# ritikasaboo13/Quantized-GEMM-for-Transformer-Inference

Measured on AMD Instinct MI355X. Metric: int8 GEMMs/sec + achieved int8-MFMA TOPS%, M=N=K=4096, 1/2/4/8 MI355X, higher is better.
Workload: dtype int8

## Files before the change

### include/qgemm.h

```cpp
#ifndef QGEMM_H_
#define QGEMM_H_

#include <stddef.h>
#include <stdint.h>

#if defined(__GNUC__)
#define QGEMM_API __attribute__((visibility("default")))
#else
#define QGEMM_API
#endif

#ifdef __cplusplus
extern "C" {
#endif

QGEMM_API int op_mm_quantize(const float *A, const float *B, float *C, int m, int n, int k);

QGEMM_API int op_mm_quantize_ex(const float *A, int64_t a_stride_h, int64_t a_stride_w,
                      const float *B, int64_t b_stride_h, int64_t b_stride_w,
                      float *C, int64_t c_stride_h, int64_t c_stride_w,
                      int m, int n, int k, float range, void *stream);

QGEMM_API size_t op_mm_quantize_workspace_size(int m, int n, int k);
QGEMM_API int op_mm_quantize_ws(const float *A, int64_t a_stride_h, int64_t a_stride_w,
// ... 33 lines not shown
QGEMM_API int qgemm_linear_dt(const void *X, int x_dtype, int64_t x_stride_h, int m, int k, const void *packed_w, int n,
                    const float *bias, int relu, void *Y, int y_dtype, int64_t y_stride_h,
                    void *workspace, size_t ws_bytes, void *stream);
QGEMM_API int qgemm_softmax_rows(const float *S, float *P, int64_t rows, int w, float scale, void *stream);
QGEMM_API int qgemm_softmax_rows_causal(const float *S, float *P, int64_t rows, int w, float scale, int seq_q,
                              int q_pos0, void *stream);
QGEMM_API int qgemm_add_layernorm_rows(const float *A, const float *B, float *Y, int64_t rows, int w, void *stream);
QGEMM_API int qgemm_encoder_create(int d_model, int n_heads, int d_ff, int n_blocks, int max_seq, uint64_t seed,
                         void **encoder);
QGEMM_API int qgemm_encoder_forward(void *encoder, const float *X, float *Y, int seq, void *stream);
QGEMM_API int qgemm_encoder_destroy(void *encoder);

QGEMM_API size_t qgemm_attention_workspace_size(int seq_q, int seq_kv, int n_heads, int d_k);
QGEMM_API int qgemm_attention(const float *Q, int64_t q_stride_h, const float *K, int64_t k_stride_h,
                    const float *V, int64_t v_stride_h, float *O, int64_t o_stride_h,
                    int seq_q, int seq_kv, int n_heads, int d_k, float scale,
                    void *workspace, size_t ws_bytes, void *stream);
QGEMM_API int qgemm_attention_causal(const float *Q, int64_t q_stride_h, const float *K, int64_t k_stride_h,
                           const float *V, int64_t v_stride_h, float *O, int64_t o_stride_h,
                           int seq_q, int seq_kv, int n_heads, int d_k, float scale, int q_pos0,
                           void *workspace, size_t ws_bytes, void *stream);
QGEMM_API int qgemm_attention_plan(int seq_q, int seq_kv, int n_heads, int d_k, const char **kernel);

QGEMM_API int qgemm_decoder_create(int d_model, int n_heads, int d_ff, int n_blocks, int max_seq, int max_enc_seq,
                         uint64_t seed, void **decoder);
enum { QGEMM_DECODER_CAUSAL = 1, QGEMM_DECODER_KV_CACHE = 8 };
QGEMM_API int qgemm_decoder_create_ex(int d_model, int n_heads, int d_ff, int n_blocks, int max_seq, int max_enc_seq,
                            uint64_t seed, int flags, void **decoder);
QGEMM_API int qgemm_decoder_forward(void *decoder, const float *X, const float *enc_out, float *Y, int seq, int enc_seq,
                          void *stream);
QGEMM_API int qgemm_decoder_begin(void *decoder, const float *enc_out, int enc_seq, void *stream);
QGEMM_API int qgemm_decoder_step(void *decoder, const float *X, float *Y, int pos, int n, void *stream);
QGEMM_API int qgemm_decoder_destroy(void *decoder);

QGEMM_API size_t qgemm_mm_outlier_workspace_size(int m, int n, int k);
QGEMM_API int qgemm_mm_outlier(const float *A, const float *B, float *C, int m, int n, int k, float threshold,
                     void *workspace, size_t ws_bytes, void *stream);
QGEMM_API int qgemm_outlier_count(int k, const void *workspace, int *count);

QGEMM_API size_t qgemm_linear_outlier_workspace_size(int m, int n, int k);
QGEMM_API int qgemm_linear_outlier(const float *X, int64_t x_stride_h, int m, int k, const void *packed_w, int n,
                         const float *bias, int relu, float threshold, float *Y, int64_t y_stride_h,
                         void *workspace, size_t ws_bytes, void *stream);

QGEMM_API int qgemm_error_stats(const float *C, const float *O, int64_t count, int reference_order, double *stats,
                      void *stream);

QGEMM_API int qgemm_fill_uniform(float *dst, int64_t count, uint64_t seed, float lo, float hi, void *stream);

QGEMM_API int qgemm_set_gemm_events(void *start_event, void *stop_event);
QGEMM_API int qgemm_set_event_mode(int mode);

QGEMM_API int qgemm_gemm_plan(int m, int n, int k, int *tile, const char **kernel);

QGEMM_API const char *qgemm_version(void);

#ifdef __cplusplus
}
#endif

#endif
```

### include/qgemm_dist.h

```cpp
#ifndef QGEMM_DIST_H_
#define QGEMM_DIST_H_

#include <stddef.h>
#include <stdint.h>

#include "qgemm.h"

#ifdef __cplusplus
extern "C" {
#endif

#define QGEMM_COMM_ID_BYTES 128

QGEMM_API int qgemm_shard_rows(int m, int world, int rank, int *m0, int *rows);

QGEMM_API int op_mm_quantize_shard(const float *A, const float *B, float *C, int m, int n, int k, int world,
                                   int rank, void *stream);

QGEMM_API int qgemm_comm_unique_id(void *id_out );
QGEMM_API int qgemm_comm_init_rank(void **comm, int world, const void *id, int rank);
QGEMM_API int qgemm_comm_init_all(void **comms, int ndev, const int *devices);
QGEMM_API int qgemm_comm_destroy(void *comm);
QGEMM_API int qgemm_comm_count(void *comm, int *count);
QGEMM_API int qgemm_comm_user_rank(void *comm, int *rank);

QGEMM_API int qgemm_allgather_rows(float *C, int m, int n, int world, int rank, void *comm, void *stream);
QGEMM_API int qgemm_allgather_plan(int m, int n, int world, int64_t *first, int64_t *count, int *root, int max_ops);

QGEMM_API int qgemm_allgather_chunk_plan(int m, int n, int world, int chunks, int64_t *first, int64_t *count,
                                         int *root, int max_ops);
QGEMM_API size_t op_mm_quantize_shard_pipelined_workspace_size(int m, int n, int k, int world, int chunks);
QGEMM_API int op_mm_quantize_shard_pipelined(const float *A, const float *B, float *C, int m, int n, int k, int world,
                                             int rank, int chunks, void *comm, void *workspace, size_t ws_bytes,
                                             void *stream, void *gather_stream);

typedef struct qgemm_coll_op {
    int rank;
    int root;
    int64_t send_off;
    int64_t recv_off;
    int64_t count;
} qgemm_coll_op;

QGEMM_API int qgemm_node_allgather_plan(int m, int n, int ndev, qgemm_coll_op *ops, int max_ops);

QGEMM_API int qgemm_node_mm_quantize(const float *const *A, const float *const *B, float *const *C, int m, int n,
                                     int k, int ndev, const int *devices, void *const *comms,
                                     void *const *streams, int mode);

#ifdef __cplusplus
}
#endif

#endif
```

### quantized-gemm-for-transformer-inference_amd/__init__.py

```python
from __future__ import annotations

import ctypes
import os
import subprocess
import threading

PKG_DIR = os.path.dirname(os.path.abspath(__file__))
REPO_DIR = os.path.dirname(PKG_DIR)
LIB_PATH = os.path.join(PKG_DIR, "build", "libqgemm.so")
HEADER_PATH = os.path.join(REPO_DIR, "include", "qgemm.h")
DIST_LIB_PATH = os.path.join(PKG_DIR, "build", "libqgemm_dist.so")
DIST_HEADER_PATH = os.path.join(REPO_DIR, "include", "qgemm_dist.h")

DEFAULT_RANGE = 127.0
ROW_PAD = 256
K_PAD = 128

EXPORTED_SYMBOLS = (
    "op_mm_quantize",
    "op_mm_quantize_ex",
    "op_mm_quantize_workspace_size",
    "op_mm_quantize_ws",
    "qgemm_packed_size",
    "qgemm_pack_a",
    "qgemm_pack_b",
    "qgemm_mm_packed",
    "qgemm_mm_packed_i32",
    "qgemm_mm_fp32",
    "qgemm_error_stats",
    "qgemm_linear_workspace_size",
    "qgemm_linear",
    "qgemm_pack_a_dt",
    "qgemm_mm_packed_dt",
    "qgemm_linear_dt",
    "op_mm_quantize_prepacked",
    "op_mm_quantize_prepacked_workspace_size",
    "op_mm_quantize_prepacked_ws",
    "qgemm_softmax_rows",
    "qgemm_softmax_rows_causal",
    "qgemm_add_layernorm_rows",
    "qgemm_encoder_create",
    "qgemm_encoder_forward",
    "qgemm_encoder_destroy",
    "qgemm_attention_workspace_size",
    "qgemm_attention",
    "qgemm_attention_causal",
    "qgemm_attention_plan",
    "qgemm_decoder_create",
    "qgemm_decoder_create_ex",
    "qgemm_decoder_forward",
    "qgemm_decoder_begin",
    "qgemm_decoder_step",
    "qgemm_decoder_destroy",
    "qgemm_mm_outlier_workspace_size",
    "qgemm_mm_outlier",
    "qgemm_outlier_count",
    "qgemm_linear_outlier_workspace_size",
    "qgemm_linear_outlier",
    "qgemm_set_gemm_events",
    "qgemm_set_event_mode",
    "qgemm_fill_uniform",
    "qgemm_gemm_plan",
    "qgemm_version",
)

DIST_EXPORTED_SYMBOLS = (
    "qgemm_shard_rows",
    "op_mm_quantize_shard",
    "qgemm_comm_unique_id",
    "qgemm_comm_init_rank",
    "qgemm_comm_init_all",
    "qgemm_comm_destroy",
    "qgemm_comm_count",
    "qgemm_comm_user_rank",
    "qgemm_allgather_rows",
    "qgemm_allgather_plan",
    "qgemm_allgather_chunk_plan",
    "op_mm_quantize_shard_pipelined_workspace_size",
    "op_mm_quantize_shard_pipelined",
    "qgemm_node_allgather_plan",
    "qgemm_node_mm_quantize",
)
COMM_ID_BYTES = 128

HIP_ERROR_INVALID_VALUE = 1
QGEMM_F32, QGEMM_BF16 = 0, 1
QGEMM_DECODER_CAUSAL = 1
QGEMM_DECODER_KV_CACHE = 8

_lock = threading.Lock()
_lib = None
_dist = None


class QGemmError(RuntimeError):

    def __init__(self, fn: str, code: int):
        super().__init__(f"{fn} failed with hipError_t {code}")
        self.code = code


def build(verbose: bool = False) -> str:
    out = None if verbose else subprocess.DEVNULL
    jobs = str(min(8, os.cpu_count() or 1))
    subprocess.run(["make", "-C", PKG_DIR, "-j", jobs, "all"], check=True, stdout=out)
    return LIB_PATH


def load() -> ctypes.CDLL:
    global _lib
    with _lock:
        if _lib is not None:
            return _lib
        if not os.path.exists(LIB_PATH):
            raise RuntimeError(f"qgemm HIP library not built: {LIB_PATH} missing (run build())")
        L = ctypes.CDLL(LIB_PATH)
        i64, i32, f32, vp, sz = ctypes.c_int64, ctypes.c_int, ctypes.c_float, ctypes.c_void_p, ctypes.c_size_t
        L.op_mm_quantize.argtypes = [vp, vp, vp, i32, i32, i32]
        L.op_mm_quantize.restype = i32
        L.op_mm_quantize_ex.argtypes = [vp, i64, i64, vp, i64, i64, vp, i64, i64, i32, i32, i32, f32, vp]
        L.op_mm_quantize_ex.restype = i32
        L.op_mm_quantize_workspace_size.argtypes = [i32, i32, i32]
        L.op_mm_quantize_workspace_size.restype = sz
        L.op_mm_quantize_ws.argtypes = [vp, i64, i64, vp, i64, i64, vp, i64, i64, i32, i32, i32, f32, vp, sz, vp]
        L.op_mm_quantize_ws.restype = i32
        L.qgemm_packed_size.argtypes = [i32, i32]
        L.qgemm_packed_size.restype = sz
        L.qgemm_pack_a.argtypes = [vp, i64, i64, i32, i32, f32, vp, vp]
        L.qgemm_pack_a.restype = i32
        L.qgemm_pack_b.argtypes = [vp, i64, i64, i32, i32, f32, vp, vp]
        L.qgemm_pack_b.restype = i32
        L.qgemm_mm_packed.argtypes = [vp, vp, vp, i64, i64, i32, i32, i32, f32, vp]
# ... 21 lines not shown
        L.op_mm_quantize_prepacked_ws.argtypes = [vp, i64, vp, vp, i64, i32, i32, i32, vp, sz, vp]
        L.op_mm_quantize_prepacked_ws.restype = i32
        L.qgemm_softmax_rows.argtypes = [vp, vp, i64, i32, f32, vp]
        L.qgemm_softmax_rows.restype = i32
        L.qgemm_softmax_rows_causal.argtypes = [vp, vp, i64, i32, f32, i32, i32, vp]
        L.qgemm_softmax_rows_causal.restype = i32
        L.qgemm_add_layernorm_rows.argtypes = [vp, vp, vp, i64, i32, vp]
        L.qgemm_add_layernorm_rows.restype = i32
        L.qgemm_encoder_create.argtypes = [i32, i32, i32, i32, i32, ctypes.c_uint64, ctypes.POINTER(vp)]
        L.qgemm_encoder_create.restype = i32
        L.qgemm_encoder_forward.argtypes = [vp, vp, vp, i32, vp]
        L.qgemm_encoder_forward.restype = i32
        L.qgemm_encoder_destroy.argtypes = [vp]
        L.qgemm_encoder_destroy.restype = i32
        L.qgemm_attention_workspace_size.argtypes = [i32, i32, i32, i32]
        L.qgemm_attention_workspace_size.restype = sz
        L.qgemm_attention.argtypes = [vp, i64, vp, i64, vp, i64, vp, i64, i32, i32, i32, i32, f32, vp, sz, vp]
        L.qgemm_attention.restype = i32
        L.qgemm_attention_causal.argtypes = [vp, i64, vp, i64, vp, i64, vp, i64, i32, i32, i32, i32, f32, i32, vp, sz,
                                             vp]
        L.qgemm_attention_causal.restype = i32
        L.qgemm_decoder_create_ex.argtypes = [i32, i32, i32, i32, i32, i32, ctypes.c_uint64, i32, ctypes.POINTER(vp)]
        L.qgemm_decoder_create_ex.restype = i32
        L.qgemm_decoder_create.argtypes = [i32, i32, i32, i32, i32, i32, ctypes.c_uint64, ctypes.POINTER(vp)]
        L.qgemm_decoder_create.restype = i32
        L.qgemm_decoder_forward.argtypes = [vp, vp, vp, vp, i32, i32, vp]
        L.qgemm_decoder_forward.restype = i32
        L.qgemm_decoder_begin.argtypes = [vp, vp, i32, vp]
        L.qgemm_decoder_begin.restype = i32
        L.qgemm_decoder_step.argtypes = [vp, vp, vp, i32, i32, vp]
        L.qgemm_decoder_step.restype = i32
        L.qgemm_attention_plan.argtypes = [i32, i32, i32, i32, ctypes.POINTER(ctypes.c_char_p)]
        L.qgemm_attention_plan.restype = i32
        L.qgemm_decoder_destroy.argtypes = [vp]
        L.qgemm_decoder_destroy.restype = i32
        L.qgemm_mm_outlier_workspace_size.argtypes = [i32, i32, i32]
        L.qgemm_mm_outlier_workspace_size.restype = sz
        L.qgemm_mm_outlier.argtypes = [vp, vp, vp, i32, i32, i32, f32, vp, sz, vp]
        L.qgemm_mm_outlier.restype = i32
        L.qgemm_outlier_count.argtypes = [i32, vp, ctypes.POINTER(i32)]
        L.qgemm_outlier_count.restype = i32
        L.qgemm_linear_outlier_workspace_size.argtypes = [i32, i32, i32]
        L.qgemm_linear_outlier_workspace_size.restype = sz
        L.qgemm_linear_outlier.argtypes = [vp, i64, i32, i32, vp, i32, vp, i32, f32, vp, i64, vp, sz, vp]
        L.qgemm_linear_outlier.restype = i32
        L.qgemm_fill_uniform.argtypes = [vp, i64, ctypes.c_uint64, f32, f32, vp]
        L.qgemm_fill_uniform.restype = i32
        L.qgemm_set_gemm_events.argtypes = [vp, vp]
        L.qgemm_set_gemm_events.restype = i32
        L.qgemm_set_event_mode.argtypes = [i32]
        L.qgemm_set_event_mode.restype = i32
        L.qgemm_gemm_plan.argtypes = [i32, i32, i32, ctypes.POINTER(ctypes.c_int), ctypes.POINTER(ctypes.c_char_p)]
        L.qgemm_gemm_plan.restype = i32
        L.qgemm_version.argtypes = []
        L.qgemm_version.restype = ctypes.c_char_p
        _lib = L
        return L


def load_dist() -> ctypes.CDLL:
    global _dist
    load()
    with _lock:
        if _dist is not None:
            return _dist
        if not os.path.exists(DIST_LIB_PATH):
            raise RuntimeError(f"qgemm multi-GPU library not built: {DIST_LIB_PATH} missing (run build())")
        D = ctypes.CDLL(DIST_LIB_PATH)
        i32, vp = ctypes.c_int, ctypes.c_void_p
        D.qgemm_shard_rows.argtypes = [i32, i32, i32, ctypes.POINTER(i32), ctypes.POINTER(i32)]
        D.qgemm_shard_rows.restype = i32
        D.op_mm_quantize_shard.argtypes = [vp, vp, vp, i32, i32, i32, i32, i32, vp]
        D.op_mm_quantize_shard.restype = i32
        D.qgemm_comm_unique_id.argtypes = [vp]
        D.qgemm_comm_unique_id.restype = i32
        D.qgemm_comm_init_rank.argtypes = [ctypes.POINTER(vp), i32, vp, i32]
        D.qgemm_comm_init_rank.restype = i32
        D.qgemm_comm_init_all.argtypes = [ctypes.POINTER(vp), i32, ctypes.POINTER(i32)]
        D.qgemm_comm_init_all.restype = i32
        D.qgemm_comm_destroy.argtypes = [vp]
        D.qgemm_comm_destroy.restype = i32
        D.qgemm_comm_count.argtypes = [vp, ctypes.POINTER(i32)]
        D.qgemm_comm_count.restype = i32
        D.qgemm_comm_user_rank.argtypes = [vp, ctypes.POINTER(i32)]
        D.qgemm_comm_user_rank.restype = i32
        D.qgemm_allgather_rows.argtypes = [vp, i32, i32, i32, i32, vp, vp]
        D.qgemm_allgather_rows.restype = i32
        i64p = ctypes.POINTER(ctypes.c_int64)
        D.qgemm_allgather_plan.argtypes = [i32, i32, i32, i64p, i64p, ctypes.POINTER(i32), i32]
        D.qgemm_allgather_plan.restype = i32
        D.qgemm_allgather_chunk_plan.argtypes = [i32, i32, i32, i32, i64p, i64p, ctypes.POINTER(i32), i32]
        D.qgemm_allgather_chunk_plan.restype = i32
        D.op_mm_quantize_shard_pipelined_workspace_size.argtypes = [i32, i32, i32, i32, i32]
        D.op_mm_quantize_shard_pipelined_workspace_size.restype = ctypes.c_size_t
        D.op_mm_quantize_shard_pipelined.argtypes = [vp, vp, vp, i32, i32, i32, i32, i32, i32, vp, vp, ctypes.c_size_t,
                                                     vp, vp]
        D.op_mm_quantize_shard_pipelined.restype = i32
        D.qgemm_node_allgather_plan.argtypes = [i32, i32, i32, ctypes.POINTER(CollOp), i32]
        D.qgemm_node_allgather_plan.restype = i32
        D.qgemm_node_mm_quantize.argtypes = [vp, vp, vp, i32, i32, i32, i32, ctypes.POINTER(i32), vp, vp, i32]
        D.qgemm_node_mm_quantize.restype = i32
        _dist = D
        return D


def shard_rows(m: int, world: int, rank: int) -> tuple:
    m0, rows = ctypes.c_int(), ctypes.c_int()
    _check("qgemm_shard_rows", load_dist().qgemm_shard_rows(m, world, rank, ctypes.byref(m0), ctypes.byref(rows)))
    return m0.value, rows.value


class CollOp(ctypes.Structure):
    _fields_ = [("rank", ctypes.c_int), ("root", ctypes.c_int), ("send_off", ctypes.c_int64),
                ("recv_off", ctypes.c_int64), ("count", ctypes.c_int64)]


def node_allgather_plan(m: int, n: int, ndev: int) -> list:
    D = load_dist()
    cnt = D.qgemm_node_allgather_plan(m, n, ndev, None, 0)
    if cnt < 0:
        raise QGemmError("qgemm_node_allgather_plan", -cnt)
    ops = (CollOp * max(1, cnt))()
    got = D.qgemm_node_allgather_plan(m, n, ndev, ops, cnt)
    if got != cnt:
        raise QGemmError("qgemm_node_allgather_plan", -got if got < 0 else 1)
    return [(o.rank, o.root, o.send_off, o.recv_off, o.count) for o in ops[:cnt]]


def allgather_plan(m: int, n: int, world: int) -> list:
    cap = max(1, world)
    first, count, root = (ctypes.c_int64 * cap)(), (ctypes.c_int64 * cap)(), (ctypes.c_int * cap)()
    ops = load_dist().qgemm_allgather_plan(m, n, world, first, count, root, cap)
    if ops < 0:
        raise QGemmError("qgemm_allgather_plan", -ops)
    return [(first[i], count[i], root[i]) for i in range(ops)]


def allgather_chunk_plan(m: int, n: int, world: int, chunks: int) -> list:
    D = load_dist()
    cnt = D.qgemm_allgather_chunk_plan(m, n, world, chunks, None, None, None, 0)
    if cnt < 0:
        raise QGemmError("qgemm_allgather_chunk_plan", -cnt)
    cap = max(1, cnt)
    first, count, root = (ctypes.c_int64 * cap)(), (ctypes.c_int64 * cap)(), (ctypes.c_int * cap)()
    got = D.qgemm_allgather_chunk_plan(m, n, world, chunks, first, count, root, cap)
    if got != cnt:
        raise QGemmError("qgemm_allgather_chunk_plan", -got if got < 0 else 1)
    return [(first[i], count[i], root[i]) for i in range(cnt)]


# ... 578 lines not shown
```

### quantized-gemm-for-transformer-inference_amd/csrc/api.hip

```cpp
#include <map>
#include <mutex>
#include <thread>
#include <stdio.h>

#include "../../include/qgemm.h"
#include "qgemm_internal.h"

using namespace qgemm;

namespace {

constexpr float kDefaultRange = 127.0f;

int err(hipError_t e) { return (int)e; }

bool dims_ok(int m, int n, int k) { return m >= 0 && n >= 0 && k >= 1; }

hipError_t pack_vectors(const float *src, int64_t row_stride, int64_t elem_stride, int rows, int len, float range,
                        PackedView out, hipStream_t stream) {
    if (elem_stride == 1) return launch_pack_rows(src, row_stride, 1, rows, len, range, out, stream);
    if (row_stride == 1 && len > 1) return launch_pack_cols(src, elem_stride, len, rows, range, out, stream);
    return launch_pack_rows(src, row_stride, elem_stride, rows, len, range, out, stream);
}

hipError_t pack_vectors(const bf16_t *src, int64_t row_stride, int64_t elem_stride, int rows, int len, float range,
                        PackedView out, hipStream_t stream) {
    return launch_pack_rows(src, row_stride, elem_stride, rows, len, range, out, stream);
}

bool dtype_ok(int t) { return t == QGEMM_F32 || t == QGEMM_BF16; }

hipError_t pack_vectors(const void *src, int dtype, int64_t row_stride, int64_t elem_stride, int rows, int len,
                        float range, PackedView out, hipStream_t stream) {
    return dtype == QGEMM_BF16
               ? pack_vectors(static_cast<const bf16_t *>(src), row_stride, elem_stride, rows, len, range, out, stream)
               : pack_vectors(static_cast<const float *>(src), row_stride, elem_stride, rows, len, range, out, stream);
}

enum CacheUse { kUseWorkspace = 0, kUseSplitK = 1, kUseErrorStats = 2 };
constexpr int kMaxCachedStreams = 8;
struct CacheKey {
    int dev;
    hipStream_t stream;
    std::thread::id thread;
    int use;
    bool operator<(const CacheKey &o) const {
        if (dev != o.dev) return dev < o.dev;
        if (stream != o.stream) return stream < o.stream;
        if (thread != o.thread) return thread < o.thread;
        return use < o.use;
    }
};
// ... 31 lines not shown
    if (e != hipSuccess) return e;
    const std::thread::id th = stream == hipStreamPerThread ? std::this_thread::get_id() : std::thread::id();
    std::lock_guard<std::mutex> lk(g_cache_mu);
    const CacheKey key{dev, stream, th, use};
    const bool fresh = g_cache.find(key) == g_cache.end();
    CachedBuf &w = g_cache[key];
    w.last_use = ++g_cache_clock;
    if (fresh && (e = evict_cached(dev, use, key)) != hipSuccess) return e;
    if (w.bytes < need) {
        if (w.ptr) {
            if ((e = hipStreamSynchronize(stream)) != hipSuccess) return e;
            if ((e = hipFree(w.ptr)) != hipSuccess) return e;
            w.ptr = nullptr;
            w.bytes = 0;
        }
        const size_t grow = need + headroom;
        if ((e = hipMalloc(&w.ptr, grow)) != hipSuccess) return e;
        if (zero_new && (e = hipMemset(w.ptr, 0, grow)) != hipSuccess) return e;
        w.bytes = grow;
    }
    *out = w.ptr;
    return hipSuccess;
}

hipError_t cached_workspace(size_t need, hipStream_t stream, void **out) {
    return cached_buffer(need, stream, kUseWorkspace, false, need / 8 , out);
}

size_t align256(size_t x) { return (x + 255) & ~(size_t)255; }

struct ChainWorkspace {
    size_t scratch_bytes;
    size_t a, b;
    size_t end;
    ChainWorkspace(int m, int n, int k)
        : scratch_bytes(gemm_scratch_bytes(m, n, k)),
          a(align256(scratch_bytes)),
          b(a + align256(packed_bytes(m, k))),
          end(b + align256(packed_bytes(n, k))) {}
};

hipError_t cached_scratch(size_t need, hipStream_t stream, int use, void **out) {
    return cached_buffer(need, stream, use, true, 0, out);
}

hipError_t mm_packed_impl(const void *packed_a, const void *packed_b, void *C, int64_t c_stride_h,
                          int64_t c_stride_w, int m, int n, int k, float range, void *scratch, size_t scratch_bytes,
                          hipStream_t stream, bool tickets_zeroed = false, bool c_bf16 = false) {
    const float inv_r2 = 1.0f / (range * range);
    return launch_gemm_dequant(packed_view(packed_a, m, k), packed_view(packed_b, n, k), C, c_stride_h, c_stride_w, m,
                               n, inv_r2, scratch, scratch_bytes, stream, nullptr, false, tickets_zeroed, c_bf16);
}

}

extern "C" {

size_t qgemm_packed_size(int rows, int k) {
    if (rows < 0 || k < 1) return 0;
    return packed_bytes(rows, k);
}

size_t op_mm_quantize_workspace_size(int m, int n, int k) {
    if (!dims_ok(m, n, k)) return 0;
    return ChainWorkspace(m, n, k).end;
}

int qgemm_pack_a(const float *A, int64_t a_stride_h, int64_t a_stride_w, int m, int k, float range, void *packed_a,
                 void *stream) {
    return qgemm_pack_a_dt(A, QGEMM_F32, a_stride_h, a_stride_w, m, k, range, packed_a, stream);
}

int qgemm_pack_b(const float *B, int64_t b_stride_h, int64_t b_stride_w, int k, int n, float range, void *packed_b,
                 void *stream) {
    if (!B || !packed_b || n < 0 || k < 1) return err(hipErrorInvalidValue);
    if (n == 0) return 0;
    return err(pack_vectors(B, b_stride_w, b_stride_h, n, k, range, packed_view(packed_b, n, k),
                            static_cast<hipStream_t>(stream)));
}

int qgemm_mm_packed(const void *packed_a, const void *packed_b, float *C, int64_t c_stride_h, int64_t c_stride_w,
                    int m, int n, int k, float range, void *stream) {
    return qgemm_mm_packed_dt(packed_a, packed_b, C, QGEMM_F32, c_stride_h, c_stride_w, m, n, k, range, stream);
}

int qgemm_mm_packed_i32(const void *packed_a, const void *packed_b, int32_t *Acc, int m, int n, int k, void *stream) {
    if (!packed_a || !packed_b || !Acc || !dims_ok(m, n, k)) return err(hipErrorInvalidValue);
    if (m == 0 || n == 0) return 0;
    return err(launch_gemm_i32(packed_view(packed_a, m, k), packed_view(packed_b, n, k), Acc, m, n,
                               static_cast<hipStream_t>(stream)));
}

int op_mm_quantize_ws(const float *A, int64_t a_stride_h, int64_t a_stride_w, const float *B, int64_t b_stride_h,
                      int64_t b_stride_w, float *C, int64_t c_stride_h, int64_t c_stride_w, int m, int n, int k,
                      float range, void *workspace, size_t ws_bytes, void *stream) {
    if (!A || !B || !C || !dims_ok(m, n, k)) return err(hipErrorInvalidValue);
    if (m == 0 || n == 0) return 0;
    const ChainWorkspace ws(m, n, k);
    if (!workspace || ws_bytes < ws.end) return err(hipErrorInvalidValue);
    char *scratch = static_cast<char *>(workspace);
    char *pa = scratch + ws.a, *pb = scratch + ws.b;
    hipStream_t s = static_cast<hipStream_t>(stream);
    auto gemm = [&](bool tickets_zeroed) {
        return err(mm_packed_impl(pa, pb, C, c_stride_h, c_stride_w, m, n, k, range, scratch, ws.scratch_bytes, s,
                                  tickets_zeroed));
    };
    uint32_t *tickets = reinterpret_cast<uint32_t *>(scratch);
    const int ntickets = (int)(gemm_ticket_bytes(m, n, k) / 4);
    if (a_stride_w == 1 && b_stride_w == 1 && k > 1) {
        const PackedView va = packed_view(pa, m, k), vb = packed_view(pb, n, k);
        hipError_t e = launch_pack_single_pass(A, a_stride_h, m, k, va, B, b_stride_h, n, vb, range, s, tickets, ntickets);
        if (e == hipSuccess) return gemm(true);
        if (e != hipErrorNotSupported) return err(e);
        e = launch_pack_two_pass(A, a_stride_h, m, k, va, B, b_stride_h, n, vb, range, s, tickets, ntickets);
        if (e == hipSuccess) return gemm(true);
        if (e != hipErrorNotSupported) return err(e);
    }
    int rc = qgemm_pack_a(A, a_stride_h, a_stride_w, m, k, range, pa, stream);
    if (rc) return rc;
    rc = qgemm_pack_b(B, b_stride_h, b_stride_w, k, n, range, pb, stream);
    if (rc) return rc;
    return gemm(false);
}

int op_mm_quantize_ex(const float *A, int64_t a_stride_h, int64_t a_stride_w, const float *B, int64_t b_stride_h,
                      int64_t b_stride_w, float *C, int64_t c_stride_h, int64_t c_stride_w, int m, int n, int k,
                      float range, void *stream) {
    if (!A || !B || !C || !dims_ok(m, n, k)) return err(hipErrorInvalidValue);
    if (m == 0 || n == 0) return 0;
    const size_t need = op_mm_quantize_workspace_size(m, n, k);
    void *ws = nullptr;
    hipError_t e = cached_workspace(need, static_cast<hipStream_t>(stream), &ws);
    if (e != hipSuccess) return err(e);
    return op_mm_quantize_ws(A, a_stride_h, a_stride_w, B, b_stride_h, b_stride_w, C, c_stride_h, c_stride_w, m, n, k,
                             range, ws, need, stream);
}

int op_mm_quantize(const float *A, const float *B, float *C, int m, int n, int k) {
    return op_mm_quantize_ex(A, k, 1, B, n, 1, C, n, 1, m, n, k, kDefaultRange, nullptr);
}

int qgemm_mm_fp32(const float *A, int64_t a_stride_h, int64_t a_stride_w, const float *B, int64_t b_stride_h,
                  int64_t b_stride_w, float *C, int64_t c_stride_h, int64_t c_stride_w, int m, int n, int k,
                  void *stream) {
    if (!A || !B || !C || !dims_ok(m, n, k)) return err(hipErrorInvalidValue);
    if (m == 0 || n == 0) return 0;
    return err(launch_mm_f32(A, a_stride_h, a_stride_w, B, b_stride_h, b_stride_w, C, c_stride_h, c_stride_w, m, n, k,
                             static_cast<hipStream_t>(stream)));
}

int qgemm_error_stats(const float *C, const float *O, int64_t count, int reference_order, double *stats,
                      void *stream) {
    if (!C || !O || !stats || count < 1) return err(hipErrorInvalidValue);
    hipStream_t s = static_cast<hipStream_t>(stream);
    void *scratch = nullptr;
    hipError_t e = cached_scratch(error_stats_scratch_bytes(), s, kUseErrorStats, &scratch);
    if (e != hipSuccess) return err(e);
    return err(launch_error_stats(C, O, count, reference_order != 0, stats, scratch, s));
}

int qgemm_linear(const float *X, int64_t x_stride_h, int m, int k, const void *packed_w, int n, const float *bias,
                 int relu, float *Y, int64_t y_stride_h, void *workspace, size_t ws_bytes, void *stream) {
// ... 282 lines not shown
```

### quantized-gemm-for-transformer-inference_amd/csrc/dist.cpp

```cpp
#include <hip/hip_runtime.h>
#include <rccl/rccl.h>

#include <vector>

#include "../../include/qgemm_dist.h"

namespace {

int nccl_rc(ncclResult_t r) { return r == ncclSuccess ? 0 : 1000 + (int)r; }

}

extern "C" {

int qgemm_shard_rows(int m, int world, int rank, int *m0, int *rows) {
    if (m < 0 || world < 1 || rank < 0 || rank >= world || !m0 || !rows) return (int)hipErrorInvalidValue;
    const int q = m / world, r = m % world;
    *m0 = rank * q + (rank < r ? rank : r);
    *rows = q + (rank < r ? 1 : 0);
    return 0;
}

int op_mm_quantize_shard(const float *A, const float *B, float *C, int m, int n, int k, int world, int rank,
                         void *stream) {
    int m0 = 0, rows = 0;
    const int e = qgemm_shard_rows(m, world, rank, &m0, &rows);
    if (e) return e;
    if (!A || !B || !C || n < 0 || k < 1) return (int)hipErrorInvalidValue;
    if (rows == 0) return 0;
    return op_mm_quantize_ex(A + (int64_t)m0 * k, k, 1, B, n, 1, C + (int64_t)m0 * n, n, 1, rows, n, k, 127.0f,
                             stream);
}

int qgemm_comm_unique_id(void *id_out) {
    if (!id_out) return (int)hipErrorInvalidValue;
    return nccl_rc(ncclGetUniqueId(static_cast<ncclUniqueId *>(id_out)));
}

int qgemm_comm_init_rank(void **comm, int world, const void *id, int rank) {
    if (!comm || !id || world < 1 || rank < 0 || rank >= world) return (int)hipErrorInvalidValue;
    ncclUniqueId uid;
    __builtin_memcpy(&uid, id, sizeof(uid));
    ncclComm_t c = nullptr;
    const int rc = nccl_rc(ncclCommInitRank(&c, world, uid, rank));
    *comm = c;
    return rc;
}

int qgemm_comm_init_all(void **comms, int ndev, const int *devices) {
    if (!comms || ndev < 1) return (int)hipErrorInvalidValue;
    return nccl_rc(ncclCommInitAll(reinterpret_cast<ncclComm_t *>(comms), ndev, devices));
}

int qgemm_comm_destroy(void *comm) {
    if (!comm) return 0;
    return nccl_rc(ncclCommDestroy(static_cast<ncclComm_t>(comm)));
}

int qgemm_comm_count(void *comm, int *count) {
    if (!comm || !count) return (int)hipErrorInvalidValue;
    return nccl_rc(ncclCommCount(static_cast<ncclComm_t>(comm), count));
}

int qgemm_comm_user_rank(void *comm, int *rank) {
    if (!comm || !rank) return (int)hipErrorInvalidValue;
    return nccl_rc(ncclCommUserRank(static_cast<ncclComm_t>(comm), rank));
}

int qgemm_allgather_plan(int m, int n, int world, int64_t *first, int64_t *count, int *root, int max_ops) {
    if (m < 0 || n < 0 || world < 1 || max_ops < 0 || (max_ops > 0 && (!first || !count || !root)))
        return -(int)hipErrorInvalidValue;
    if (world == 1 || m == 0 || n == 0) return 0;
    if (m % world == 0) {
        if (max_ops < 1) return -(int)hipErrorInvalidValue;
        first[0] = 0;
        count[0] = (int64_t)(m / world) * n;
        root[0] = -1;
        return 1;
    }
    int ops = 0;
    for (int r = 0; r < world; ++r) {
        int m0 = 0, rows = 0;
        qgemm_shard_rows(m, world, r, &m0, &rows);
        if (rows == 0) continue;
        if (ops >= max_ops) return -(int)hipErrorInvalidValue;
        first[ops] = (int64_t)m0 * n;
        count[ops] = (int64_t)rows * n;
        root[ops] = r;
        ++ops;
    }
    return ops;
}

namespace {

int chunk_plan(int m, int n, int world, int chunks, int64_t *first, int64_t *count, int *root, int *chunk_of,
               int max_ops) {
    const bool query = first == nullptr;
    int ops = 0;
    for (int c = 0; c < chunks; ++c)
        for (int r = 0; r < world; ++r) {
            int m0 = 0, rows = 0, c0 = 0, crows = 0;
            qgemm_shard_rows(m, world, r, &m0, &rows);
            qgemm_shard_rows(rows, chunks, c, &c0, &crows);
            if (crows == 0 || n == 0) continue;
            if (!query) {
                if (ops >= max_ops) return -(int)hipErrorInvalidValue;
                first[ops] = (int64_t)(m0 + c0) * n;
                count[ops] = (int64_t)crows * n;
                root[ops] = r;
                if (chunk_of) chunk_of[ops] = c;
            }
            ++ops;
        }
    return ops;
}

}

int qgemm_allgather_chunk_plan(int m, int n, int world, int chunks, int64_t *first, int64_t *count, int *root,
                               int max_ops) {
    if (m < 0 || n < 0 || world < 1 || chunks < 1 || max_ops < 0) return -(int)hipErrorInvalidValue;
    if (max_ops == 0 || !first || !count || !root) return chunk_plan(m, n, world, chunks, nullptr, nullptr, nullptr,
                                                                     nullptr, 0);
    return chunk_plan(m, n, world, chunks, first, count, root, nullptr, max_ops);
}

size_t op_mm_quantize_shard_pipelined_workspace_size(int m, int n, int k, int world, int chunks) {
    if (m < 0 || n < 1 || k < 1 || world < 1 || chunks < 1) return 0;
    const int rows = (m + world - 1) / world, crows = (rows + chunks - 1) / chunks;
    const size_t pb = (qgemm_packed_size(n, k) + 255) / 256 * 256;
    return pb + op_mm_quantize_prepacked_workspace_size(crows > 0 ? crows : 1, n, k);
}

int op_mm_quantize_shard_pipelined(const float *A, const float *B, float *C, int m, int n, int k, int world, int rank,
                                   int chunks, void *comm, void *workspace, size_t ws_bytes, void *stream,
                                   void *gather_stream) {
    int m0 = 0, rows = 0;
    const int e = qgemm_shard_rows(m, world, rank, &m0, &rows);
    if (e) return e;
    if (!A || !B || !C || n < 1 || k < 1 || chunks < 1 || !workspace || (world > 1 && !comm))
        return (int)hipErrorInvalidValue;
    if (ws_bytes < op_mm_quantize_shard_pipelined_workspace_size(m, n, k, world, chunks))
        return (int)hipErrorInvalidValue;
    const int nops = chunk_plan(m, n, world, chunks, nullptr, nullptr, nullptr, nullptr, 0);
    std::vector<int64_t> first((size_t)nops + 1), count((size_t)nops + 1);
    std::vector<int> root((size_t)nops + 1), chunk_of((size_t)nops + 1);
    if (nops > 0 &&
        chunk_plan(m, n, world, chunks, first.data(), count.data(), root.data(), chunk_of.data(), nops) != nops)
        return (int)hipErrorInvalidValue;
    hipStream_t s = static_cast<hipStream_t>(stream), g = static_cast<hipStream_t>(gather_stream);
    ncclComm_t cm = static_cast<ncclComm_t>(comm);
    const size_t pb_bytes = (qgemm_packed_size(n, k) + 255) / 256 * 256;
    char *ws = static_cast<char *>(workspace);
    int rc = qgemm_pack_b(B, n, 1, k, n, 127.0f, ws, s);
    hipEvent_t ev = nullptr;
    hipError_t he = hipEventCreateWithFlags(&ev, hipEventDisableTiming);
    if (he != hipSuccess && rc == 0) rc = (int)he;
    int op = 0;
    for (int c = 0; c < chunks; ++c) {
        int c0 = 0, crows = 0;
        qgemm_shard_rows(rows, chunks, c, &c0, &crows);
        if (crows > 0 && rc == 0)
            rc = op_mm_quantize_prepacked_ws(A + (int64_t)(m0 + c0) * k, k, ws, C + (int64_t)(m0 + c0) * n, n, crows,
                                             n, k, ws + pb_bytes, ws_bytes - pb_bytes, s);
        const int o0 = op;
        while (op < nops && chunk_of[(size_t)op] == c) ++op;
        if (!cm || op == o0) continue;
        if (rc == 0 &&
            ((he = hipEventRecord(ev, s)) != hipSuccess || (he = hipStreamWaitEvent(g, ev, 0)) != hipSuccess))
            rc = (int)he;
        ncclResult_t r = ncclGroupStart();
        for (int i = o0; i < op && r == ncclSuccess; ++i)
            r = ncclBroadcast(C + first[(size_t)i], C + first[(size_t)i], (size_t)count[(size_t)i], ncclFloat32,
                              root[(size_t)i], cm, g);
        const ncclResult_t r2 = ncclGroupEnd();
        if (rc == 0) rc = nccl_rc(r != ncclSuccess ? r : r2);
    }
    if (rc == 0 && cm && op > 0) {
        if ((he = hipEventRecord(ev, g)) != hipSuccess || (he = hipStreamWaitEvent(s, ev, 0)) != hipSuccess)
            rc = (int)he;
    }
    if (ev) (void)hipEventDestroy(ev);
    return rc;
}

int qgemm_node_allgather_plan(int m, int n, int ndev, qgemm_coll_op *ops, int max_ops) {
    if (m < 0 || n < 0 || ndev < 1 || max_ops < 0 || (max_ops > 0 && !ops)) return -(int)hipErrorInvalidValue;
    std::vector<int64_t> first((size_t)ndev), count((size_t)ndev);
    std::vector<int> root((size_t)ndev);
    const int nplan = qgemm_allgather_plan(m, n, ndev, first.data(), count.data(), root.data(), ndev);
    if (nplan < 0) return nplan;
    const int64_t total = (int64_t)nplan * ndev;
    if (ops == nullptr) return (int)total;
    if (total > max_ops) return -(int)hipErrorInvalidValue;
    int o = 0;
    for (int r = 0; r < ndev; ++r)
        for (int i = 0; i < nplan; ++i, ++o) {
            qgemm_coll_op &op = ops[o];
            op.rank = r;
            op.root = root[i];
            op.count = count[i];
            op.recv_off = first[i];
            op.send_off = root[i] < 0 ? first[i] + (int64_t)r * count[i] : first[i];
        }
    return o;
}

namespace {

ncclResult_t issue(const qgemm_coll_op &op, float *C, ncclComm_t c, hipStream_t s) {
    if (op.root < 0) return ncclAllGather(C + op.send_off, C + op.recv_off, (size_t)op.count, ncclFloat32, c, s);
    return ncclBroadcast(C + op.send_off, C + op.recv_off, (size_t)op.count, ncclFloat32, op.root, c, s);
}

}

int qgemm_allgather_rows(float *C, int m, int n, int world, int rank, void *comm, void *stream) {
    if (!C || !comm || m < 0 || n < 0 || world < 1 || rank < 0 || rank >= world) return (int)hipErrorInvalidValue;
    ncclComm_t c = static_cast<ncclComm_t>(comm);
    hipStream_t s = static_cast<hipStream_t>(stream);
    std::vector<int64_t> first((size_t)world), count((size_t)world);
    std::vector<int> root((size_t)world);
    const int ops = qgemm_allgather_plan(m, n, world, first.data(), count.data(), root.data(), world);
    if (ops < 0) return -ops;
    if (ops == 0) return 0;
    qgemm_coll_op op{};
    op.rank = rank;
    if (ops == 1 && root[0] < 0) {
        op.root = -1, op.count = count[0], op.recv_off = first[0], op.send_off = first[0] + (int64_t)rank * count[0];
        return nccl_rc(issue(op, C, c, s));
    }
    ncclResult_t r = ncclGroupStart();
    for (int i = 0; i < ops && r == ncclSuccess; ++i) {
        op.root = root[i], op.count = count[i], op.recv_off = first[i], op.send_off = first[i];
        r = issue(op, C, c, s);
// ... 45 lines not shown
```

Baseline: 12020.

## Batch pipelined event records with event pool and add row-chunked large-M GEMM path

Reworks the pipelined shard GEMM so that compute for up to 16 chunks is issued first, each recording a cached per-device event, and only then are the broadcast groups issued, instead of interleaving record/wait/broadcast per chunk with a freshly created event. It also adds a row-chunked quantize+GEMM path that packs B once and streams A in 8192-row chunks when M is at least 32768, reusing smaller workspace. For the 4096 test shape the chunked path will not trigger, so the main effect is fewer event creations and a different launch order, at the cost of a global mutex held during the call.

```diff
diff --git a/include/qgemm.h b/include/qgemm.h
--- a/include/qgemm.h
+++ b/include/qgemm.h
@@ -109,6 +109,10 @@
 QGEMM_API int qgemm_set_event_mode(int mode);
 
 QGEMM_API int qgemm_gemm_plan(int m, int n, int k, int *tile, const char **kernel);
+QGEMM_API int qgemm_chunk_plan(int rows, int n, int k, int *chunk_rows);
+QGEMM_API size_t qgemm_mm_quantize_chunked_workspace_size(int m, int n, int k, int chunk_rows);
+QGEMM_API int qgemm_mm_quantize_chunked(const float *A, const float *B, float *C, int m, int n, int k,
+                                        int chunk_rows, void *workspace, size_t ws_bytes, void *stream);
 
 QGEMM_API const char *qgemm_version(void);
 
diff --git a/include/qgemm_dist.h b/include/qgemm_dist.h
--- a/include/qgemm_dist.h
+++ b/include/qgemm_dist.h
@@ -34,6 +34,23 @@
                                              int rank, int chunks, void *comm, void *workspace, size_t ws_bytes,
                                              void *stream, void *gather_stream);
 
+#define QGEMM_PIPE_EVENT_POOL 16
+#define QGEMM_PIPE_COMPUTE 0
+#define QGEMM_PIPE_RECORD 1
+#define QGEMM_PIPE_WAIT 2
+#define QGEMM_PIPE_GROUP 3
+#define QGEMM_PIPE_JOIN 4
+typedef struct qgemm_pipe_step {
+    int kind;
+    int chunk;
+    int slot;
+} qgemm_pipe_step;
+QGEMM_API int qgemm_pipelined_schedule(int m, int n, int world, int rank, int chunks, int gather,
+                                       qgemm_pipe_step *steps, int max_steps);
+#define QGEMM_PIPE_TEST_GATHER_WORLD1 1
+#define QGEMM_PIPE_TEST_STARVE_CHUNK1 2
+QGEMM_API int qgemm_pipelined_test_mode(int flags);
+
 typedef struct qgemm_coll_op {
     int rank;
     int root;
diff --git a/quantized-gemm-for-transformer-inference_amd/__init__.py b/quantized-gemm-for-transformer-inference_amd/__init__.py
--- a/quantized-gemm-for-transformer-inference_amd/__init__.py
+++ b/quantized-gemm-for-transformer-inference_amd/__init__.py
@@ -61,6 +61,9 @@
     "qgemm_set_event_mode",
     "qgemm_fill_uniform",
     "qgemm_gemm_plan",
+    "qgemm_chunk_plan",
+    "qgemm_mm_quantize_chunked_workspace_size",
+    "qgemm_mm_quantize_chunked",
     "qgemm_version",
 )
 
@@ -78,6 +81,8 @@
     "qgemm_allgather_chunk_plan",
     "op_mm_quantize_shard_pipelined_workspace_size",
     "op_mm_quantize_shard_pipelined",
+    "qgemm_pipelined_schedule",
+    "qgemm_pipelined_test_mode",
     "qgemm_node_allgather_plan",
     "qgemm_node_mm_quantize",
 )
@@ -205,10 +210,20 @@
         L.qgemm_set_event_mode.restype = i32
         L.qgemm_gemm_plan.argtypes = [i32, i32, i32, ctypes.POINTER(ctypes.c_int), ctypes.POINTER(ctypes.c_char_p)]
         L.qgemm_gemm_plan.restype = i32
+        L.qgemm_chunk_plan.argtypes = [i32, i32, i32, ctypes.POINTER(ctypes.c_int)]
+        L.qgemm_chunk_plan.restype = i32
+        L.qgemm_mm_quantize_chunked_workspace_size.argtypes = [i32, i32, i32, i32]
+        L.qgemm_mm_quantize_chunked_workspace_size.restype = ctypes.c_size_t
+        L.qgemm_mm_quantize_chunked.argtypes = [vp, vp, vp, i32, i32, i32, i32, vp, ctypes.c_size_t, vp]
+        L.qgemm_mm_quantize_chunked.restype = i32
         L.qgemm_version.argtypes = []
         L.qgemm_version.restype = ctypes.c_char_p
         _lib = L
         return L
+
+
+class PipeStep(ctypes.Structure):
+    _fields_ = [("kind", ctypes.c_int), ("chunk", ctypes.c_int), ("slot", ctypes.c_int)]
 
 
 def load_dist() -> ctypes.CDLL:
@@ -249,6 +264,10 @@
         D.op_mm_quantize_shard_pipelined.argtypes = [vp, vp, vp, i32, i32, i32, i32, i32, i32, vp, vp, ctypes.c_size_t,
                                                      vp, vp]
         D.op_mm_quantize_shard_pipelined.restype = i32
+        D.qgemm_pipelined_schedule.argtypes = [i32, i32, i32, i32, i32, i32, ctypes.POINTER(PipeStep), i32]
+        D.qgemm_pipelined_schedule.restype = i32
+        D.qgemm_pipelined_test_mode.argtypes = [i32]
+        D.qgemm_pipelined_test_mode.restype = i32
         D.qgemm_node_allgather_plan.argtypes = [i32, i32, i32, ctypes.POINTER(CollOp), i32]
         D.qgemm_node_allgather_plan.restype = i32
         D.qgemm_node_mm_quantize.argtypes = [vp, vp, vp, i32, i32, i32, i32, ctypes.POINTER(i32), vp, vp, i32]
diff --git a/quantized-gemm-for-transformer-inference_amd/csrc/api.hip b/quantized-gemm-for-transformer-inference_amd/csrc/api.hip
--- a/quantized-gemm-for-transformer-inference_amd/csrc/api.hip
+++ b/quantized-gemm-for-transformer-inference_amd/csrc/api.hip
@@ -1,3 +1,4 @@
+#include <algorithm>
 #include <map>
 #include <mutex>
 #include <thread>
@@ -135,9 +136,81 @@
                                n, inv_r2, scratch, scratch_bytes, stream, nullptr, false, tickets_zeroed, c_bf16);
 }
 
+constexpr int kChunkRows = 8192;
+constexpr int kChunkThresholdRows = 32768;
+
+size_t chunked_workspace_bytes(int m, int n, int k, int chunk_rows) {
+    const int last = m % chunk_rows;
+    size_t chain = ChainWorkspace(chunk_rows < m ? chunk_rows : m, n, k).b;
+    if (m > chunk_rows && last) chain = std::max(chain, ChainWorkspace(last, n, k).b);
+    return align256(packed_bytes(n, k)) + chain;
+}
+
+int plan_chunk_rows(int rows, int n, int k) {
+    if (rows < kChunkThresholdRows || n < 1 || k < 2) return rows;
+    int tile_whole = 0, tile_chunk = 0;
+    const int kp = round_up(k, kKPad);
+    if (gemm_plan_info(rows, n, kp, &tile_whole, nullptr) != 1) return rows;
+    if (gemm_plan_info(kChunkRows, n, kp, &tile_chunk, nullptr) != 1 || tile_chunk != tile_whole) return rows;
+    if (chunked_workspace_bytes(rows, n, k, kChunkRows) > ChainWorkspace(rows, n, k).end) return rows;
+    return kChunkRows;
+}
+
+int mm_quantize_chunked(const float *A, int64_t a_stride_h, const float *B, int64_t b_stride_h, float *C,
+                        int64_t c_stride_h, int64_t c_stride_w, int m, int n, int k, float range, int chunk_rows,
+                        char *ws, size_t ws_bytes, hipStream_t s) {
+    if (chunk_rows < 1 || ws_bytes < chunked_workspace_bytes(m, n, k, chunk_rows)) return err(hipErrorInvalidValue);
+    char *chain = ws + align256(packed_bytes(n, k));
+    const PackedView vb = packed_view(ws, n, k);
+    const int rows0 = m < chunk_rows ? m : chunk_rows;
+    hipError_t e = k > 1 ? launch_pack_single_pass(A, a_stride_h, rows0, k,
+                                                   packed_view(chain + ChainWorkspace(rows0, n, k).a, rows0, k), B,
+                                                   b_stride_h, n, vb, range, s, nullptr, 0)
+                         : hipErrorNotSupported;
+    const bool first_packed = e == hipSuccess;
+    if (e == hipErrorNotSupported) e = pack_vectors(B, 1, b_stride_h, n, k, range, vb, s);
+    for (int r0 = 0; r0 < m && e == hipSuccess; r0 += chunk_rows) {
+        const int rows = m - r0 < chunk_rows ? m - r0 : chunk_rows;
+        const ChainWorkspace cw(rows, n, k);
+        if (r0 > 0 || !first_packed)
+            e = pack_vectors(A + (int64_t)r0 * a_stride_h, a_stride_h, 1, rows, k, range,
+                             packed_view(chain + cw.a, rows, k), s);
+        if (e == hipSuccess)
+            e = mm_packed_impl(chain + cw.a, ws, C + (int64_t)r0 * c_stride_h, c_stride_h, c_stride_w, rows, n, k,
+                               range, chain, cw.scratch_bytes, s);
+    }
+    return err(e);
+}
+
 }
 
 extern "C" {
+
+int qgemm_chunk_plan(int rows, int n, int k, int *chunk_rows) {
+    if (rows < 0 || n < 0 || k < 1) return -(int)hipErrorInvalidValue;
+    const int cr = rows > 0 && n > 0 ? plan_chunk_rows(rows, n, k) : rows;
+    if (chunk_rows) *chunk_rows = cr;
+    return cr > 0 ? (rows + cr - 1) / cr : 1;
+}
+
+size_t qgemm_mm_quantize_chunked_workspace_size(int m, int n, int k, int chunk_rows) {
+    if (!dims_ok(m, n, k) || chunk_rows < 1) return 0;
+    return chunked_workspace_bytes(m, n, k, chunk_rows);
+}
+
+int qgemm_mm_quantize_chunked(const float *A, const float *B, float *C, int m, int n, int k, int chunk_rows,
+                              void *workspace, size_t ws_bytes, void *stream) {
+    if (!A || !B || !C || !dims_ok(m, n, k) || chunk_rows < 1) return err(hipErrorInvalidValue);
+    if (m == 0 || n == 0) return 0;
+    hipStream_t s = static_cast<hipStream_t>(stream);
+    if (!workspace) {
+        ws_bytes = chunked_workspace_bytes(m, n, k, chunk_rows);
+        hipError_t e = cached_workspace(ws_bytes, s, &workspace);
+        if (e != hipSuccess) return err(e);
+    }
+    return mm_quantize_chunked(A, k, B, n, C, n, 1, m, n, k, kDefaultRange, chunk_rows, static_cast<char *>(workspace),
+                               ws_bytes, s);
+}
 
 size_t qgemm_packed_size(int rows, int k) {
     if (rows < 0 || k < 1) return 0;
@@ -191,6 +264,10 @@
     uint32_t *tickets = reinterpret_cast<uint32_t *>(scratch);
     const int ntickets = (int)(gemm_ticket_bytes(m, n, k) / 4);
     if (a_stride_w == 1 && b_stride_w == 1 && k > 1) {
+        const int chunk_rows = plan_chunk_rows(m, n, k);
+        if (chunk_rows < m)
+            return mm_quantize_chunked(A, a_stride_h, B, b_stride_h, C, c_stride_h, c_stride_w, m, n, k, range,
+                                       chunk_rows, scratch, ws_bytes, s);
         const PackedView va = packed_view(pa, m, k), vb = packed_view(pb, n, k);
         hipError_t e = launch_pack_single_pass(A, a_stride_h, m, k, va, B, b_stride_h, n, vb, range, s, tickets, ntickets);
         if (e == hipSuccess) return gemm(true);
diff --git a/quantized-gemm-for-transformer-inference_amd/csrc/dist.cpp b/quantized-gemm-for-transformer-inference_amd/csrc/dist.cpp
--- a/quantized-gemm-for-transformer-inference_amd/csrc/dist.cpp
+++ b/quantized-gemm-for-transformer-inference_amd/csrc/dist.cpp
@@ -1,6 +1,9 @@
 #include <hip/hip_runtime.h>
 #include <rccl/rccl.h>
 
+#include <algorithm>
+#include <atomic>
+#include <mutex>
 #include <vector>
 
 #include "../../include/qgemm_dist.h"
@@ -94,43 +97,125 @@
 
 namespace {
 
-int chunk_plan(int m, int n, int world, int chunks, int64_t *first, int64_t *count, int *root, int *chunk_of,
-               int max_ops) {
+bool chunk_op(int m, int n, int world, int chunks, int c, int r, int64_t *first, int64_t *count) {
+    int m0 = 0, rows = 0, c0 = 0, crows = 0;
+    qgemm_shard_rows(m, world, r, &m0, &rows);
+    qgemm_shard_rows(rows, chunks, c, &c0, &crows);
+    if (crows == 0 || n == 0) return false;
+    if (first) *first = (int64_t)(m0 + c0) * n;
+    if (count) *count = (int64_t)crows * n;
+    return true;
+}
+
+int chunk_plan(int m, int n, int world, int chunks, int64_t *first, int64_t *count, int *root, int max_ops) {
     const bool query = first == nullptr;
     int ops = 0;
     for (int c = 0; c < chunks; ++c)
         for (int r = 0; r < world; ++r) {
-            int m0 = 0, rows = 0, c0 = 0, crows = 0;
-            qgemm_shard_rows(m, world, r, &m0, &rows);
-            qgemm_shard_rows(rows, chunks, c, &c0, &crows);
-            if (crows == 0 || n == 0) continue;
+            int64_t f = 0, cnt = 0;
+            if (!chunk_op(m, n, world, chunks, c, r, &f, &cnt)) continue;
             if (!query) {
                 if (ops >= max_ops) return -(int)hipErrorInvalidValue;
-                first[ops] = (int64_t)(m0 + c0) * n;
-                count[ops] = (int64_t)crows * n;
+                first[ops] = f;
+                count[ops] = cnt;
                 root[ops] = r;
-                if (chunk_of) chunk_of[ops] = c;
             }
             ++ops;
         }
     return ops;
 }
 
+constexpr int kEventPool = QGEMM_PIPE_EVENT_POOL;
+
+bool chunk_has_ops(int m, int n, int world, int chunks, int c) {
+    return chunk_op(m, n, world, chunks, c, 0, nullptr, nullptr);
+}
+
+extern "C++" template <class Visit>
+void walk_schedule(int m, int n, int world, int rank, int chunks, bool gather, Visit &&visit) {
+    int m0 = 0, rows = 0;
+    qgemm_shard_rows(m, world, rank, &m0, &rows);
+    auto mine = [&](int c) {
+        int c0 = 0, crows = 0;
+        qgemm_shard_rows(rows, chunks, c, &c0, &crows);
+        return crows > 0;
+    };
+    bool any_group = false;
+    for (int b = 0; b < chunks; b += kEventPool) {
+        const int e = chunks - b < kEventPool ? chunks : b + kEventPool;
+        for (int c = b; c < e; ++c) {
+            if (!mine(c)) continue;
+            visit(QGEMM_PIPE_COMPUTE, c, 0);
+            if (gather) visit(QGEMM_PIPE_RECORD, c, c - b);
+        }
+        for (int c = b; c < e && gather; ++c) {
+            if (!chunk_has_ops(m, n, world, chunks, c)) continue;
+            if (mine(c)) visit(QGEMM_PIPE_WAIT, c, c - b);
+            visit(QGEMM_PIPE_GROUP, c, 0);
+            any_group = true;
+        }
+    }
+    if (any_group) visit(QGEMM_PIPE_JOIN, chunks, kEventPool);
+}
+
+struct EventPool {
+    std::mutex mu;
+    bool ready = false;
+    hipEvent_t ev[kEventPool + 1] = {};
+};
+constexpr int kMaxDevices = 64;
+EventPool g_pools[kMaxDevices];
+
+hipError_t event_pool(EventPool **out) {
+    int dev = 0;
+    hipError_t e = hipGetDevice(&dev);
+    if (e != hipSuccess) return e;
+    if (dev < 0 || dev >= kMaxDevices) return hipErrorInvalidDevice;
+    EventPool &p = g_pools[dev];
+    std::lock_guard<std::mutex> lk(p.mu);
+    for (int i = 0; i <= kEventPool && !p.ready; ++i)
+        if (!p.ev[i] && (e = hipEventCreateWithFlags(&p.ev[i], hipEventDisableTiming)) != hipSuccess) return e;
+    p.ready = true;
+    *out = &p;
+    return hipSuccess;
+}
+
+std::atomic<int> g_test_mode{0};
+
+}
+
+int qgemm_pipelined_test_mode(int flags) { return g_test_mode.exchange(flags); }
+
+int qgemm_pipelined_schedule(int m, int n, int world, int rank, int chunks, int gather, qgemm_pipe_step *steps,
+                             int max_steps) {
+    if (m < 0 || n < 0 || world < 1 || rank < 0 || rank >= world || chunks < 1 || max_steps < 0)
+        return -(int)hipErrorInvalidValue;
+    int cnt = 0;
+    walk_schedule(m, n, world, rank, chunks, gather != 0, [&](int kind, int chunk, int slot) {
+        if (steps && cnt < max_steps) steps[cnt] = qgemm_pipe_step{kind, chunk, slot};
+        ++cnt;
+    });
+    return steps && cnt > max_steps ? -(int)hipErrorInvalidValue : cnt;
 }
 
 int qgemm_allgather_chunk_plan(int m, int n, int world, int chunks, int64_t *first, int64_t *count, int *root,
                                int max_ops) {
     if (m < 0 || n < 0 || world < 1 || chunks < 1 || max_ops < 0) return -(int)hipErrorInvalidValue;
-    if (max_ops == 0 || !first || !count || !root) return chunk_plan(m, n, world, chunks, nullptr, nullptr, nullptr,
-                                                                     nullptr, 0);
-    return chunk_plan(m, n, world, chunks, first, count, root, nullptr, max_ops);
+    if (max_ops == 0 || !first || !count || !root) return chunk_plan(m, n, world, chunks, nullptr, nullptr, nullptr, 0);
+    return chunk_plan(m, n, world, chunks, first, count, root, max_ops);
 }
 
 size_t op_mm_quantize_shard_pipelined_workspace_size(int m, int n, int k, int world, int chunks) {
     if (m < 0 || n < 1 || k < 1 || world < 1 || chunks < 1) return 0;
     const int rows = (m + world - 1) / world, crows = (rows + chunks - 1) / chunks;
     const size_t pb = (qgemm_packed_size(n, k) + 255) / 256 * 256;
-    return pb + op_mm_quantize_prepacked_workspace_size(crows > 0 ? crows : 1, n, k);
+    size_t chain = op_mm_quantize_prepacked_workspace_size(crows > 0 ? crows : 1, n, k);
+    if (crows > 1) chain = std::max(chain, op_mm_quantize_prepacked_workspace_size(crows - 1, n, k));
+    size_t need = pb + chain;
+    int plan_rows = 0;
+    if (world == 1 && qgemm_chunk_plan(rows, n, k, &plan_rows) > 1)
+        need = std::max(need, qgemm_mm_quantize_chunked_workspace_size(rows, n, k, plan_rows));
+    return need;
 }
 
 int op_mm_quantize_shard_pipelined(const float *A, const float *B, float *C, int m, int n, int k, int world, int rank,
@@ -143,45 +228,68 @@
         return (int)hipErrorInvalidValue;
     if (ws_bytes < op_mm_quantize_shard_pipelined_workspace_size(m, n, k, world, chunks))
         return (int)hipErrorInvalidValue;
-    const int nops = chunk_plan(m, n, world, chunks, nullptr, nullptr, nullptr, nullptr, 0);
-    std::vector<int64_t> first((size_t)nops + 1), count((size_t)nops + 1);
-    std::vector<int> root((size_t)nops + 1), chunk_of((size_t)nops + 1);
-    if (nops > 0 &&
-        chunk_plan(m, n, world, chunks, first.data(), count.data(), root.data(), chunk_of.data(), nops) != nops)
-        return (int)hipErrorInvalidValue;
     hipStream_t s = static_cast<hipStream_t>(stream), g = static_cast<hipStream_t>(gather_stream);
     ncclComm_t cm = static_cast<ncclComm_t>(comm);
+    const int test_mode = g_test_mode.load();
+    const bool gather = cm && (world > 1 || (test_mode & QGEMM_PIPE_TEST_GATHER_WORLD1));
+    int plan_rows = 0;
+    if (!gather && test_mode == 0 && qgemm_chunk_plan(rows, n, k, &plan_rows) > 1)
+        return qgemm_mm_quantize_chunked(A + (int64_t)m0 * k, B, C + (int64_t)m0 * n, rows, n, k, plan_rows, workspace,
+                                         ws_bytes, stream);
     const size_t pb_bytes = (qgemm_packed_size(n, k) + 255) / 256 * 256;
     char *ws = static_cast<char *>(workspace);
     int rc = qgemm_pack_b(B, n, 1, k, n, 127.0f, ws, s);
-    hipEvent_t ev = nullptr;
-    hipError_t he = hipEventCreateWithFlags(&ev, hipEventDisableTiming);
-    if (he != hipSuccess && rc == 0) rc = (int)he;
-    int op = 0;
-    for (int c = 0; c < chunks; ++c) {
-        int c0 = 0, crows = 0;
-        qgemm_shard_rows(rows, chunks, c, &c0, &crows);
-        if (crows > 0 && rc == 0)
+    EventPool *pool = nullptr;
+    if (gather) {
+        const hipError_t he = event_pool(&pool);
+        if (he != hipSuccess && rc == 0) rc = (int)he;
+    }
+    std::unique_lock<std::mutex> lk;
+    if (pool) lk = std::unique_lock<std::mutex>(pool->mu);
+    bool recorded[kEventPool] = {};
+    walk_schedule(m, n, world, rank, chunks, gather, [&](int kind, int c, int slot) {
+        hipError_t he = hipSuccess;
+        switch (kind) {
+        case QGEMM_PIPE_COMPUTE: {
+            if (rc != 0) break;
+            int c0 = 0, crows = 0;
+            qgemm_shard_rows(rows, chunks, c, &c0, &crows);
+            const size_t chain_bytes = (test_mode & QGEMM_PIPE_TEST_STARVE_CHUNK1) && c == 1 ? 0 : ws_bytes - pb_bytes;
             rc = op_mm_quantize_prepacked_ws(A + (int64_t)(m0 + c0) * k, k, ws, C + (int64_t)(m0 + c0) * n, n, crows,
-                                             n, k, ws + pb_bytes, ws_bytes - pb_bytes, s);
-        const int o0 = op;
-        while (op < nops && chunk_of[(size_t)op] == c) ++op;
-        if (!cm || op == o0) continue;
-        if (rc == 0 &&
-            ((he = hipEventRecord(ev, s)) != hipSuccess || (he = hipStreamWaitEvent(g, ev, 0)) != hipSuccess))
-            rc = (int)he;
-        ncclResult_t r = ncclGroupStart();
-        for (int i = o0; i < op && r == ncclSuccess; ++i)
-            r = ncclBroadcast(C + first[(size_t)i], C + first[(size_t)i], (size_t)count[(size_t)i], ncclFloat32,
-                              root[(size_t)i], cm, g);
-        const ncclResult_t r2 = ncclGroupEnd();
-        if (rc == 0) rc = nccl_rc(r != ncclSuccess ? r : r2);
-    }
-    if (rc == 0 && cm && op > 0) {
-        if ((he = hipEventRecord(ev, g)) != hipSuccess || (he = hipStreamWaitEvent(s, ev, 0)) != hipSuccess)
-            rc = (int)he;
-    }
-    if (ev) (void)hipEventDestroy(ev);
+                                             n, k, ws + pb_bytes, chain_bytes, s);
+            break;
+        }
+        case QGEMM_PIPE_RECORD:
+            if (rc != 0 || !pool) break;
+            if ((he = hipEventRecord(pool->ev[slot], s)) != hipSuccess) rc = (int)he;
+            else recorded[slot] = true;
+            break;
+        case QGEMM_PIPE_WAIT:
+            if (!recorded[slot]) break;
+            recorded[slot] = false;
+            if ((he = hipStreamWaitEvent(g, pool->ev[slot], 0)) != hipSuccess && rc == 0) rc = (int)he;
+            break;
+        case QGEMM_PIPE_GROUP: {
+            ncclResult_t r = ncclGroupStart();
+            for (int o = 0; o < world && r == ncclSuccess; ++o) {
+                int64_t first = 0, count = 0;
+                if (!chunk_op(m, n, world, chunks, c, o, &first, &count)) continue;
+                r = ncclBroadcast(C + first, C + first, (size_t)count, ncclFloat32, o, cm, g);
+            }
+            const ncclResult_t r2 = ncclGroupEnd();
+            if (rc == 0) rc = nccl_rc(r != ncclSuccess ? r : r2);
+            break;
+        }
+        case QGEMM_PIPE_JOIN:
+            if (pool) {
+                if ((he = hipEventRecord(pool->ev[slot], g)) == hipSuccess) he = hipStreamWaitEvent(s, pool->ev[slot], 0);
+            } else {
+                he = hipStreamSynchronize(g);
+            }
+            if (he != hipSuccess && rc == 0) rc = (int)he;
+            break;
+        }
+    });
     return rc;
 }
 
```

Result: no change. 11990 (-0.2%).
